# hyperplane-lab/ACL-GAN

Hardware: AMD Instinct MI355X
Metric: training images/sec at 256x256 (gen+dis step) (higher is better)
Workload: dtype fp32

## Files before the change

acl-gan_amd/csrc/conv_fast.hip:

```cpp
#include "conv_fast_common.h"
#include <cstring>

namespace aclgan {
namespace {


constexpr int BK = 16;
constexpr int WG_MAX_CHUNK = 1024 + 16;
constexpr int LDK = BK + 4;

template <int T, bool KC>
__device__ __forceinline__ void read_frags(const float* __restrict__ tile, int ld, int base, int lane, float (&f)[T][8]) {
    const int l31 = lane & 31, kh = lane >> 5;
    if (KC) {
#pragma unroll
        for (int t = 0; t < T; ++t) {
            const f32x4* p = reinterpret_cast<const f32x4*>(tile + (base + t * 32 + l31) * LDK + kh * 8);
            const f32x4 a = p[0], b = p[1];
            f[t][0] = a.x; f[t][1] = a.y; f[t][2] = a.z; f[t][3] = a.w;
            f[t][4] = b.x; f[t][5] = b.y; f[t][6] = b.z; f[t][7] = b.w;
        }
    } else {
#pragma unroll
        for (int ks = 0; ks < 8; ++ks)
#pragma unroll
            for (int t = 0; t < T; ++t) f[t][ks] = tile[(kh * 8 + ks) * ld + base + t * 32 + l31];
    }
}

template <int TM, int TN>
__device__ __forceinline__ void mfma_step(const float (&fa)[TM][8], const float (&fb)[TN][8], int ks, f32x16 (&acc)[TM][TN]) {
#pragma unroll
    for (int i = 0; i < TM; ++i)
#pragma unroll
        for (int j = 0; j < TN; ++j) acc[i][j] = __builtin_amdgcn_mfma_f32_32x32x2f32(fa[i][ks], fb[j][ks], acc[i][j], 0, 0, 0);
}

#define ACL_GEMM_MAINLOOP(TM_, TN_, AKC_, BKC_, KBEG_, NK_, AS_, BS_, ASTR_, BSTR_, LDA_, LDB_, AM_, BN_) \
    do {                                                                                                 \
        const int nk__ = (NK_), kb__ = (KBEG_);                                                          \
        fetch(kb__);                                                                                     \
        stage(0, true);                                                                                  \
        fetch(kb__ + min(1, nk__ - 1));                                                                  \
        __syncthreads();                                                                                 \
        for (int kt = 0; kt < nk__; ++kt) {                                                              \
            const int cur = kt & 1;                                                                      \
            float fa[TM_][8], fb[TN_][8];                                                                \
            read_frags<TM_, AKC_>((AS_) + cur * (ASTR_), (LDA_), (AM_), lane, fa);                       \
            read_frags<TN_, BKC_>((BS_) + cur * (BSTR_), (LDB_), (BN_), lane, fb);                       \
            if (!(AKC_) && !(BKC_)) __builtin_amdgcn_sched_barrier(0);    \
            mfma_step<TM_, TN_>(fa, fb, 0, acc);                                                         \
            stage(cur ^ 1, kt + 1 < nk__);                                                               \
            fetch(kb__ + min(kt + 2, nk__ - 1));                                                         \
            __builtin_amdgcn_sched_barrier(0x6);    \
            mfma_step<TM_, TN_>(fa, fb, 1, acc);                                                         \
            mfma_step<TM_, TN_>(fa, fb, 2, acc);                                                         \
            mfma_step<TM_, TN_>(fa, fb, 3, acc);                                                         \
            mfma_step<TM_, TN_>(fa, fb, 4, acc);                                                         \
            mfma_step<TM_, TN_>(fa, fb, 5, acc);                                                         \
            mfma_step<TM_, TN_>(fa, fb, 6, acc);                                                         \
            mfma_step<TM_, TN_>(fa, fb, 7, acc);                                                         \
            __syncthreads();                                                                             \
        }                                                                                                \
    } while (0)



template <int WM, int WN, int TM, int TN, int OCC = 1>
__global__ void __launch_bounds__(WM * WN * 64, OCC) conv_fwd_fast_kernel(FwdFP pk) {
    constexpr int BM = WM * TM * 32, BN = WN * TN * 32, NT = WM * WN * 64;
    constexpr int RP = NT / 4;
    FwdFP p = pk;
    if (pk.fsl) {
        const long long f = blockIdx.y;
        p.x += (pk.fsx_mod ? f % pk.fsx_mod : f) * pk.fs_x; p.w += f * pk.fs_w; p.y += f * pk.fs_y;
    }
    constexpr int A_IT = BM / RP, B_IT = (BN + RP - 1) / RP;
    __shared__ __attribute__((aligned(16))) float smem[2 * (BM + BN) * LDK];
    __shared__ int ro[BM];
    float* As = smem;
    float* Bs = smem + 2 * BM * LDK;

    const int tid = threadIdx.x, lane = tid & 63, wave = tid >> 6;
    const int wm = wave / WN, wn = wave % WN;
    const int tile = xcd_map(blockIdx.x, p.nwg);
    const int m0 = (tile / p.tiles_n) * BM, n0 = (tile % p.tiles_n) * BN;
    const int q = tid & 3, r0 = tid >> 2;
    const int phase = p.phases ? (int)blockIdx.z : 0;
    const float* wbase = p.w + (size_t)phase * p.Co * p.K;

    for (int r = tid; r < BM; r += NT) {
        int b, oy, ox, o = -1;
        if (fwd_row(p, m0 + r, b, oy, ox)) {
            if (p.phases) o = (b * p.Hf + 2 * (oy + 1) + (phase >> 1)) * p.Wf + 2 * (ox + 1) + (phase & 1);
            else o = (b * p.Ho + oy) * p.Wo + ox;
        }
        ro[r] = o;
    }
    int ay[A_IT], ax[A_IT], ab[A_IT];
#pragma unroll
    for (int i = 0; i < A_IT; ++i) {
        int b = 0, oy = 0, ox = 0;
        if (!fwd_row(p, m0 + r0 + i * RP, b, oy, ox)) { b = 0; oy = 0; ox = 0; }
        ay[i] = oy * p.s - p.p; ax[i] = ox * p.s - p.p; ab[i] = b * p.Hi * p.Wi;
    }
    int wo[B_IT];
#pragma unroll
    for (int i = 0; i < B_IT; ++i) wo[i] = min(n0 + r0 + i * RP, p.Co - 1) * p.K + q * 4;

    const int cpt = p.Ci >> 4;
    int aoff[A_IT];
    f32x4 ra[A_IT], rb[B_IT];
    int f_tap = -1;

    auto fetch = [&](int kt) __attribute__((always_inline)) {
        const int tap = kt / cpt, cc = kt - tap * cpt;
        if (tap != f_tap) {
            f_tap = tap;
            const int ky = tap / p.k, kx = tap - ky * p.k;
#pragma unroll
            for (int i = 0; i < A_IT; ++i) {
                const int iy = refl(ay[i] + ky, p.Hu) >> p.up;
                const int ix = refl(ax[i] + kx, p.Wu) >> p.up;
                aoff[i] = (ab[i] + iy * p.Wi + ix) * p.Ci + q * 4;
            }
        }
#pragma unroll
        for (int i = 0; i < A_IT; ++i) ra[i] = *reinterpret_cast<const f32x4*>(p.x + (size_t)aoff[i] + cc * 16);
#pragma unroll
        for (int i = 0; i < B_IT; ++i)
            if (BN % RP == 0 || r0 + i * RP < BN) rb[i] = *reinterpret_cast<const f32x4*>(wbase + (size_t)wo[i] + kt * 16);
    };
    auto stage = [&](int buf, bool real) __attribute__((always_inline)) {
        float* a = As + buf * BM * LDK;
        float* b = Bs + buf * BN * LDK;
#pragma unroll
        for (int i = 0; i < A_IT; ++i) *reinterpret_cast<f32x4*>(a + (r0 + i * RP) * LDK + q * 4) = ra[i];
#pragma unroll
        for (int i = 0; i < B_IT; ++i)
            if (BN % RP == 0 || r0 + i * RP < BN) *reinterpret_cast<f32x4*>(b + (r0 + i * RP) * LDK + q * 4) = rb[i];
    };

    f32x16 acc[TM][TN];
#pragma unroll
    for (int i = 0; i < TM; ++i)
#pragma unroll
        for (int j = 0; j < TN; ++j)
#pragma unroll
            for (int r = 0; r < 16; ++r) acc[i][j][r] = 0.f;

    const int nk_all = p.K / BK;
    const int kbeg = p.phases ? 0 : blockIdx.z * p.nkz, nk = p.phases ? nk_all : min(p.nkz, nk_all - kbeg);
    if (nk <= 0) return;
    const bool split = !p.phases && gridDim.z > 1;
    ACL_GEMM_MAINLOOP(TM, TN, true, true, kbeg, nk, As, Bs, BM * LDK, BN * LDK, LDK, LDK, wm * TM * 32, wn * TN * 32);

    const int l31 = lane & 31, lh = lane >> 5;
#pragma unroll
    for (int j = 0; j < TN; ++j) {
        const int n = n0 + wn * TN * 32 + j * 32 + l31;
        if (n >= p.Co) continue;
        const float bv = p.bias ? p.bias[n] : 0.f;
#pragma unroll
        for (int i = 0; i < TM; ++i) {
#pragma unroll
            for (int r = 0; r < 16; ++r) {
                const int rl = wm * TM * 32 + i * 32 + (r & 3) + 8 * (r >> 2) + 4 * lh;
                const int o = ro[rl];
                if (o >= 0) {
                    if (split && p.part) p.part[((size_t)blockIdx.z * p.rows + m0 + rl) * p.Co + n] = acc[i][j][r];
                    else if (split) atomicAdd(p.y + (size_t)o * p.Co + n, acc[i][j][r] + ((p.ring > 0 && blockIdx.z == 0) ? bv : 0.f));
                    else p.y[(size_t)o * p.Co + n] = act_apply(acc[i][j][r] + bv, p.act);
                }
            }
        }
    }
}


template <int WM, int WN, int TM, int TN>
int launch_fwd_fast(const ConvGeom& g, FwdFP p, hipStream_t st) {
    constexpr int BM = WM * TM * 32, BN = WN * TN * 32;
    p.tiles_n = cdiv(g.Co, BN);
    int rows = p.M;
    if (p.ring > 0) rows = p.B * (p.Ho * p.Wo - std::max(0, p.Ho - 2 * p.ring) * std::max(0, p.Wo - 2 * p.ring));
    p.nwg = cdiv(rows, BM) * p.tiles_n;
    if (p.phases) {
        hipLaunchKernelGGL((conv_fwd_fast_kernel<WM, WN, TM, TN>), dim3(p.nwg, 1, 4), dim3(WM * WN * 64), 0, st, p);
        ACL_CHECK_LAUNCH("conv_fwd_fast_kernel(phases)");
        return ACLGAN_OK;
    }
    int splits = 1;
    fwd_split_plan(rows, g.Co, g.K, BK, &splits, &p.nkz);
    p.rows = rows;
    if (splits > 1 && p.part != nullptr) {
        hipLaunchKernelGGL((conv_fwd_fast_kernel<WM, WN, TM, TN>), dim3(p.nwg, 1, splits), dim3(WM * WN * 64), 0, st, p);
        ACL_CHECK_LAUNCH("conv_fwd_fast_kernel(split)");
        hipLaunchKernelGGL(fwd_split_finish_kernel, dim3((int)std::min<int64_t>(cdiv64((int64_t)rows * std::max(1, g.Co / 4), 256), 4096)), dim3(256), 0, st, p, splits);
        ACL_CHECK_LAUNCH("fwd_split_finish_kernel");
        return ACLGAN_OK;
    }
    p.part = nullptr;
    const int nk = g.K / BK;
    if (p.ring > 0 && (p.act != ACLGAN_ACT_NONE || g.Co % 4 != 0)) splits = 1, p.nkz = nk;
    if (sw(SW_DETERMINISTIC)) splits = 1, p.nkz = nk;
    if (splits > 1 && p.ring > 0) {
        hipLaunchKernelGGL(ring_zero_kernel, dim3(cdiv(rows * (g.Co / 4), 256)), dim3(256), 0, st, p, rows);
        ACL_CHECK_LAUNCH("ring_zero_kernel");
    } else if (splits > 1) {
        hipError_t e = hipMemsetAsync(p.y, 0, (size_t)g.M * g.Co * sizeof(float), st);
        if (e != hipSuccess) return hip_fail(e, "memset y");
    }
    hipLaunchKernelGGL((conv_fwd_fast_kernel<WM, WN, TM, TN>), dim3(p.nwg, 1, splits), dim3(WM * WN * 64), 0, st, p);
    ACL_CHECK_LAUNCH("conv_fwd_fast_kernel");
    if (splits > 1 && p.ring == 0) {
        const int64_t n = (int64_t)g.M * g.Co;
        hipLaunchKernelGGL(bias_act_kernel, dim3((int)std::min<int64_t>(cdiv64(n, 256), 4096)), dim3(256), 0, st, p.y, p.bias, g.Co, p.act, n);
        ACL_CHECK_LAUNCH("bias_act_kernel");
    }
    return ACLGAN_OK;
}


template <int WM, int WN, int TM, int TN>
__global__ void __launch_bounds__(WM * WN * 64) conv_dgrad_fast_kernel(DgFP p) {
    constexpr int BM = WM * TM * 32, BN = WN * TN * 32, NT = WM * WN * 64;
    constexpr int RP = NT / 4;
    constexpr int A_IT = BM / RP;
    constexpr int LDB = BN + 4, NVB = BN / 4;
    constexpr int B_IT = (BK * NVB + NT - 1) / NT;
    __shared__ __attribute__((aligned(16))) float smem[2 * (BM * LDK + BK * LDB)];
    __shared__ int ri_o[BM];
    __shared__ unsigned long long tap_mask;
    __shared__ int tap_list[64];
    float* As = smem;
    float* Bs = smem + 2 * BM * LDK;

    const int tid = threadIdx.x, lane = tid & 63, wave = tid >> 6;
    const int wm = wave / WN, wn = wave % WN;
    const int tile = xcd_map(blockIdx.x, p.nwg);
    const int m0 = (tile / p.tiles_n) * BM;
    const int n0 = (tile % p.tiles_n) * BN;
    const int cls = blockIdx.z / p.ksplit, slice = blockIdx.z - cls * p.ksplit;
    const int cy = cls / p.s, cx = cls % p.s;
    const int Tx = (p.k - cx + p.s - 1) / p.s, Ty = (p.k - cy + p.s - 1) / p.s;
    const int q = tid & 3, r0 = tid >> 2;

    int ylo, yhi, xlo, xhi;
    dg_box(p, cy, cx, ylo, yhi, xlo, xhi);
    const bool compact = p.mode == 2 && Ty * Tx <= 64;
    if (tid == 0) tap_mask = 0ull;
    __syncthreads();
    for (int r = tid; r < BM; r += NT) {
        int oo = -1, b, y2, x2;
        if (dg_row(p, m0 + r, ylo, yhi, xlo, xhi, b, y2, x2)) {
            const int py = y2 * p.s + cy, px = x2 * p.s + cx;
            if (compact && py < p.Hp && px < p.Wp) {
                unsigned long long mk = 0ull;
                for (int t = 0; t < Ty * Tx; ++t) {
                    const int ty = t / Tx, tx = t - ty * Tx;
                    const int oy = y2 - ty, ox = x2 - tx;
                    bool ok = (unsigned)oy < (unsigned)p.Ho && (unsigned)ox < (unsigned)p.Wo;
                    if (p.band > 0) ok = ok && (oy < 2 || oy >= p.Ho - 2 || ox < 2 || ox >= p.Wo - 2);
                    if (ok) mk |= 1ull << t;
                }
                if (mk) atomicOr(&tap_mask, mk);
            }
            if (py < p.Hp && px < p.Wp) {
                if (p.mode == 0 || p.ringpad) oo = (b * p.Hp + py) * p.Wp + px;
                else oo = (b * p.Hd + (refl(py - p.pad, p.Hi) >> p.upshift)) * p.Wd + (refl(px - p.pad, p.Wi) >> p.upshift);
            }
        }
        ri_o[r] = oo;
    }
    int ntap = Ty * Tx;
    if (compact) {
        __syncthreads();
        if (tid == 0) {
            int n = 0;
            for (int t = 0; t < Ty * Tx; ++t)
                if ((tap_mask >> t) & 1ull) tap_list[n++] = t;
            tap_list[63] = n;
        }
        __syncthreads();
        ntap = tap_list[63];
        if (ntap == 0) return;
    }
    int ay[A_IT], ax[A_IT], ab[A_IT];
#pragma unroll
    for (int i = 0; i < A_IT; ++i) {
        int b = 0, y2 = 0, x2 = 0;
        if (!dg_row(p, m0 + r0 + i * RP, ylo, yhi, xlo, xhi, b, y2, x2)) { b = 0; y2 = 0; x2 = 0; }
        ay[i] = y2; ax[i] = x2; ab[i] = b;
    }
    int bo[B_IT];
#pragma unroll
    for (int i = 0; i < B_IT; ++i) {
        const int idx = tid + i * NT;
        const int krow = idx / NVB, nc = idx - krow * NVB;
        const int n = n0 + nc * 4;
        bo[i] = krow * p.k * p.k * p.Ci + (n < p.Ci ? n : 0);
    }
    const int cpt = p.Co >> 4;
    int aoff[A_IT];
    f32x4 ra[A_IT], rb[B_IT];
    float za[A_IT];
    int f_tap = -1, tapoff = 0;

    auto fetch = [&](int kt) __attribute__((always_inline)) {
        const int tq = kt / cpt, cc = kt - tq * cpt;
        if (tq != f_tap) {
            f_tap = tq;
            const int t = compact ? tap_list[tq] : tq;
            const int ty = t / Tx, tx = t - ty * Tx;
            tapoff = ((cy + p.s * ty) * p.k + (cx + p.s * tx)) * p.Ci;
#pragma unroll
            for (int i = 0; i < A_IT; ++i) {
                const int oy = ay[i] - ty, ox = ax[i] - tx;
                const bool ok = (unsigned)oy < (unsigned)p.Ho && (unsigned)ox < (unsigned)p.Wo;
                bool okk = ok;
                if (p.band > 0) okk = ok && (oy < 2 || oy >= p.Ho - 2 || ox < 2 || ox >= p.Wo - 2);
                const int dpix = p.dyv ? (ab[i] * p.Hf + 2 * (oy + 1) + p.py) * p.Wf + 2 * (ox + 1) + p.px
                                       : (ab[i] * p.Ho + oy) * p.Wo + ox;
                aoff[i] = okk ? dpix * p.Co + q * 4 : -1;
            }
        }
#pragma unroll
        for (int i = 0; i < A_IT; ++i) {
            ra[i] = *reinterpret_cast<const f32x4*>(p.dy + (size_t)(aoff[i] < 0 ? 0 : aoff[i]) + cc * 16);
            za[i] = aoff[i] < 0 ? 0.f : 1.f;
        }
#pragma unroll
        for (int i = 0; i < B_IT; ++i)
            if ((BK * NVB) % NT == 0 || tid + i * NT < BK * NVB)
                rb[i] = *reinterpret_cast<const f32x4*>(p.w + (size_t)bo[i] + tapoff + (size_t)cc * 16 * p.k * p.k * p.Ci);
    };
    auto stage = [&](int buf, bool real) __attribute__((always_inline)) {
        float* a = As + buf * BM * LDK;
        float* b = Bs + buf * BK * LDB;
#pragma unroll
        for (int i = 0; i < A_IT; ++i) *reinterpret_cast<f32x4*>(a + (r0 + i * RP) * LDK + q * 4) = ra[i] * za[i];
#pragma unroll
        for (int i = 0; i < B_IT; ++i) {
            const int idx = tid + i * NT;
            if ((BK * NVB) % NT == 0 || idx < BK * NVB) {
                const int krow = idx / NVB, nc = idx - krow * NVB;
                *reinterpret_cast<f32x4*>(b + krow * LDB + nc * 4) = rb[i];
            }
        }
    };

    f32x16 acc[TM][TN];
#pragma unroll
    for (int i = 0; i < TM; ++i)
#pragma unroll
        for (int j = 0; j < TN; ++j)
#pragma unroll
            for (int r = 0; r < 16; ++r) acc[i][j][r] = 0.f;

    const int nk_all = ntap * cpt;
    const int nkz = (nk_all + p.ksplit - 1) / p.ksplit;
    const int kbeg = slice * nkz, nk = min(nkz, nk_all - kbeg);
    if (nk <= 0) return;
    ACL_GEMM_MAINLOOP(TM, TN, true, false, kbeg, nk, As, Bs, BM * LDK, BK * LDB, LDK, LDB, wm * TM * 32, wn * TN * 32);

    const int l31 = lane & 31, lh = lane >> 5;
#pragma unroll
    for (int j = 0; j < TN; ++j) {
        const int n = n0 + wn * TN * 32 + j * 32 + l31;
        if (n >= p.Ci) continue;
#pragma unroll
        for (int i = 0; i < TM; ++i) {
#pragma unroll
            for (int r = 0; r < 16; ++r) {
                const int of = ri_o[wm * TM * 32 + i * 32 + (r & 3) + 8 * (r >> 2) + 4 * lh];
                if (of >= 0) {
                    float* o = p.dxp + (size_t)of * p.Ci + n;
                    if (p.ksplit > 1 || (p.mode == 2 && !p.ringpad)) atomicAdd(o, acc[i][j][r]);
                    else if (p.accumulate) *o += acc[i][j][r];
                    else *o = acc[i][j][r];
                }
            }
        }
    }
}

template <int WM, int WN, int TM, int TN>
int launch_dgrad_fast(const ConvGeom& g, DgFP p, hipStream_t st) {
    constexpr int BM = WM * TM * 32, BN = WN * TN * 32;
    int mmax = 0;
    for (int cy = 0; cy < g.s; ++cy)
        for (int cx = 0; cx < g.s; ++cx) {
            const int ylo = g.p > cy ? (g.p - cy + g.s - 1) / g.s : 0, xlo = g.p > cx ? (g.p - cx + g.s - 1) / g.s : 0;
            const int yhi = std::min(p.Hc - 1, (g.p + g.Hi - 1 - cy) / g.s), xhi = std::min(p.Wc - 1, (g.p + g.Wi - 1 - cx) / g.s);
            int inner = (yhi - ylo + 1) * (xhi - xlo + 1);
            if (p.band > 0) inner = std::max(0, p.Hc - 2 * p.band) * std::max(0, p.Wc - 2 * p.band);
            const int rows = p.mode == 0 ? p.Hc * p.Wc : (p.mode == 1 ? inner : p.Hc * p.Wc - inner);
            mmax = std::max(mmax, g.B * rows);
        }
    if (mmax <= 0) return ACLGAN_OK;
    p.Mc = mmax;
    p.tiles_n = cdiv(g.Ci, BN);
    p.nwg = cdiv(p.Mc, BM) * p.tiles_n;
    const int nk_min = ((g.k + g.s - 1) / g.s) * ((g.k + g.s - 1) / g.s) * (g.Co / 16);
    const int nblk = p.nwg * g.s * g.s;
    p.ksplit = 1;
    const int nk_plan = (p.mode == 2 && p.band == 0) ? std::max(g.Co / 16, nk_min / ((g.k + g.s - 1) / g.s)) : nk_min;
    if (nblk < 128 && nk_plan >= 32 && !sw(SW_DETERMINISTIC) && !p.ringpad)
        p.ksplit = max(1, min(nk_plan / 8, 512 / nblk));
    if (p.ksplit > 1 && p.mode == 0) {
        hipError_t e = hipMemsetAsync(p.dxp, 0, conv_dgrad_scratch_bytes(g), st);
        if (e != hipSuccess) return hip_fail(e, "memset dxp");
    }
    if (p.ksplit > 1 && p.mode == 1 && !p.accumulate) {
        hipError_t e = hipMemsetAsync(p.dxp, 0, (size_t)g.B * g.Hi * g.Wi * g.Ci * sizeof(float), st);
        if (e != hipSuccess) return hip_fail(e, "memset dx");
    }
    hipLaunchKernelGGL((conv_dgrad_fast_kernel<WM, WN, TM, TN>), dim3(p.nwg, 1, g.s * g.s * p.ksplit), dim3(WM * WN * 64), 0, st, p);
    ACL_CHECK_LAUNCH("conv_dgrad_fast_kernel");
    return ACLGAN_OK;
}

template <int WM, int WN, int TM, int TN>
int launch_dgrad_halo(const ConvGeom& g, DgFP p, hipStream_t st) {
    if (p.band == 0 && !p.ringpad && g.k == 3 && g.s == 1 && g.Ci % 128 == 0 && WM == 2 && WN == 2 && TM == 2 && TN == 2)
        return launch_dgrad_fast<2, 2, 1, 2>(g, p, st);
    return launch_dgrad_fast<WM, WN, TM, TN>(g, p, st);
}

template <int WM, int WN, int TM, int TN>
int dgrad_fast_all(const ConvGeom& g, DgFP p, float* dxp, float* dx, int accumulate, bool* direct, hipStream_t st) {
    if (g.up == 0 && dx != nullptr && (!sw(SW_DETERMINISTIC) || g.p == 0 || (dxp && conv_wino_ok(g)))) {
        *direct = true;
        p.dxp = dx; p.accumulate = accumulate;
        p.mode = 1;
        int rc = (dxp && conv_wino_ok(g)) ? conv_dgrad_wino_interior(g, p.dy, p.w, dx, accumulate, dxp, st)
             : (dxp && conv_s2k4_wino_ok(g, 1)) ? conv_dgrad_s2k4_wino_interior(g, p.dy, p.w, dx, accumulate, dxp, st)
                                      : launch_dgrad_fast<WM, WN, TM, TN>(g, p, st);
        if (rc) return rc;
        if (g.p > 0 && sw(SW_DETERMINISTIC)) {
            hipError_t e = hipMemsetAsync(dxp, 0, (size_t)g.B * g.Hp * g.Wp * g.Ci * sizeof(float), st);
            if (e != hipSuccess) return hip_fail(e, "memset padded grid");
            p.mode = 2; p.ringpad = 1; p.dxp = dxp; p.accumulate = 0;
            rc = launch_dgrad_fast<WM, WN, TM, TN>(g, p, st);
            if (rc) return rc;
            return conv_fold(g, dxp, dx, 1, st);
        }
        if (g.p > 0) { p.mode = 2; rc = launch_dgrad_halo<WM, WN, TM, TN>(g, p, st); }
        return rc;
    }
    *direct = false;
    p.dxp = dxp; p.mode = 0; p.accumulate = 0;
    return launch_dgrad_fast<WM, WN, TM, TN>(g, p, st);
}


template <int WM, int WN, int TM, int TN, bool ST>
__global__ void __launch_bounds__(WM * WN * 64) conv_wgrad_fast_kernel(WgFP p) {
    constexpr int BM = WM * TM * 32, BN = WN * TN * 32, NT = WM * WN * 64;
    constexpr int LDA = BM + 4, LDB = BN + 4, MVA = BM / 4, NVB = BN / 4;
    constexpr int A_IT = (BK * MVA + NT - 1) / NT, B_IT = (BK * NVB + NT - 1) / NT;
    __shared__ __attribute__((aligned(16))) float smem[2 * BK * (LDA + LDB)];
    float* As = smem;
    float* Bs = smem + 2 * BK * LDA;

    const int tid = threadIdx.x, lane = tid & 63, wave = tid >> 6;
    const int wm = wave / WN, wn = wave % WN;
    const int tile = xcd_map(blockIdx.x, p.nwg);
    const int m0 = (tile / p.tiles_n) * BM, n0 = (tile % p.tiles_n) * BN;
    const int pbeg = blockIdx.z * p.chunk;
    const int pend = min(p.P, pbeg + p.chunk);
    if (pbeg >= pend) return;
    const int phase = p.phases ? (int)blockIdx.y : 0;
    float* dwbase = p.dw + (size_t)phase * p.Co * p.Kn + (size_t)blockIdx.z * p.dw_zs;
    const int py = phase >> 1, px = phase & 1;

    __shared__ int4 pinfo[WG_MAX_CHUNK];
    const int st_tap = n0 / p.Ci, st_ky = st_tap / p.k, st_kx = st_tap - st_ky * p.k;
    for (int i = tid; i < pend - pbeg + BK; i += NT) {
        int b, oy, ox;
        wg_coord(p, min(pbeg + i, pend - 1), b, oy, ox);
        const int dyp = p.phases ? (b * p.Hf + 2 * (oy + 1) + py) * p.Wf + 2 * (ox + 1) + px : (b * p.Ho + oy) * p.Wo + ox;
        if (ST) {
            const int iy = refl(oy * p.s - p.p + st_ky, p.Hu) >> p.up, ix = refl(ox * p.s - p.p + st_kx, p.Wu) >> p.up;
            pinfo[i] = make_int4(b * p.Hi * p.Wi + iy * p.Wi + ix, 0, 0, dyp);
        } else {
            pinfo[i] = make_int4(oy * p.s - p.p, ox * p.s - p.p, b * p.Hi * p.Wi, dyp);
        }
    }
    __syncthreads();

    int a_m[A_IT], a_kr[A_IT];
#pragma unroll
    for (int i = 0; i < A_IT; ++i) {
        const int idx = tid + i * NT;
        a_kr[i] = idx / MVA;
        const int m = m0 + (idx - a_kr[i] * MVA) * 4;
        a_m[i] = m < p.Co ? m : 0;
    }
    int b_kr[B_IT], b_ci[B_IT], b_ky[B_IT], b_kx[B_IT];
#pragma unroll
    for (int i = 0; i < B_IT; ++i) {
        const int idx = tid + i * NT;
        b_kr[i] = idx / NVB;
        int n = n0 + (idx - b_kr[i] * NVB) * 4;
        if (n >= p.Kn) n = 0;
        const int tap = n / p.Ci;
        b_ci[i] = n - tap * p.Ci; b_ky[i] = tap / p.k; b_kx[i] = tap - b_ky[i] * p.k;
    }
    f32x4 ra[A_IT], rb[B_IT];
    float za[A_IT];
    const bool do_bias = p.db != nullptr && (tile % p.tiles_n) == 0;
    f32x4 bsum[A_IT];
#pragma unroll
    for (int i = 0; i < A_IT; ++i) bsum[i] = (f32x4){0.f, 0.f, 0.f, 0.f};

    auto fetch = [&](int kt) __attribute__((always_inline)) {
        const int pb = kt * BK;
#pragma unroll
        for (int i = 0; i < A_IT; ++i) {
            if ((BK * MVA) % NT != 0 && tid + i * NT >= BK * MVA) continue;
            const int pi = pb + a_kr[i];
            ra[i] = *reinterpret_cast<const f32x4*>(p.dy + (size_t)pinfo[pi].w * p.Co + a_m[i]);
            za[i] = pbeg + pi < pend ? 1.f : 0.f;
        }
#pragma unroll
        for (int i = 0; i < B_IT; ++i) {
            if ((BK * NVB) % NT != 0 && tid + i * NT >= BK * NVB) continue;
            if (ST) {
                rb[i] = *reinterpret_cast<const f32x4*>(p.x + (size_t)pinfo[pb + b_kr[i]].x * p.Ci + b_ci[i]);
            } else {
                const int4 pi = pinfo[pb + b_kr[i]];
                const int iy = refl(pi.x + b_ky[i], p.Hu) >> p.up;
                const int ix = refl(pi.y + b_kx[i], p.Wu) >> p.up;
                rb[i] = *reinterpret_cast<const f32x4*>(p.x + (size_t)(pi.z + iy * p.Wi + ix) * p.Ci + b_ci[i]);
            }
        }
    };
    auto stage = [&](int buf, bool real) __attribute__((always_inline)) {
        float* a = As + buf * BK * LDA;
        float* b = Bs + buf * BK * LDB;
#pragma unroll
        for (int i = 0; i < A_IT; ++i) {
            const int idx = tid + i * NT;
            if ((BK * MVA) % NT == 0 || idx < BK * MVA) {
                const f32x4 v = ra[i] * za[i];
                *reinterpret_cast<f32x4*>(a + a_kr[i] * LDA + (idx - a_kr[i] * MVA) * 4) = v;
                bsum[i] += v * (real ? 1.f : 0.f);
            }
        }
#pragma unroll
        for (int i = 0; i < B_IT; ++i) {
            const int idx = tid + i * NT;
            if ((BK * NVB) % NT == 0 || idx < BK * NVB) *reinterpret_cast<f32x4*>(b + b_kr[i] * LDB + (idx - b_kr[i] * NVB) * 4) = rb[i];
        }
    };

    f32x16 acc[TM][TN];
#pragma unroll
    for (int i = 0; i < TM; ++i)
#pragma unroll
        for (int j = 0; j < TN; ++j)
#pragma unroll
            for (int r = 0; r < 16; ++r) acc[i][j][r] = 0.f;

    ACL_GEMM_MAINLOOP(TM, TN, false, false, 0, (pend - pbeg + BK - 1) / BK, As, Bs, BK * LDA, BK * LDB, LDA, LDB, wm * TM * 32, wn * TN * 32);

    if (do_bias) {
        float* red = smem;
#pragma unroll
        for (int i = 0; i < A_IT; ++i) {
            const int idx = tid + i * NT;
            if ((BK * MVA) % NT == 0 || idx < BK * MVA) *reinterpret_cast<f32x4*>(red + a_kr[i] * BM + (idx - a_kr[i] * MVA) * 4) = bsum[i];
        }
        __syncthreads();
        if (tid < BM && m0 + tid < p.Co) {
            float t = 0.f;
#pragma unroll
            for (int r = 0; r < BK; ++r) t += red[r * BM + tid];
            atomicAdd(p.db + (size_t)blockIdx.z * p.db_zs + m0 + tid, t);
        }
    }
    const int l31 = lane & 31, lh = lane >> 5;
#pragma unroll
    for (int j = 0; j < TN; ++j) {
        const int n = n0 + wn * TN * 32 + j * 32 + l31;
        if (n >= p.Kn) continue;
#pragma unroll
        for (int i = 0; i < TM; ++i) {
#pragma unroll
            for (int r = 0; r < 16; ++r) {
                const int m = m0 + wm * TM * 32 + i * 32 + (r & 3) + 8 * (r >> 2) + 4 * lh;
                if (m < p.Co) {
                    atomicAdd(dwbase + (size_t)m * p.Kn + n, acc[i][j][r]);
                }
            }
        }
    }
}

constexpr int WGKC_TARGET = 768;

template <int WM, int WN, int TM, int TN>
__global__ void __launch_bounds__(WM * WN * 64) conv_wgrad_kc_kernel(WgFP pk, WgPartX xp) {
    constexpr int BM = WM * TM * 32, BN = WN * TN * 32, NT = WM * WN * 64;
    WgFP p = pk;
    if (pk.fsl) {
        const long long f = blockIdx.y;
        p.x += (pk.fsx_mod ? f % pk.fsx_mod : f) * pk.fs_x; p.dy += f * pk.fs_dy;
    }
    static_assert(BM % 64 == 0 && BN % 64 == 0 && BM + BN <= NT, "one staging unit (4 channels x 4 pixels) per thread, wave-uniform roles");
    constexpr int CH = 1024;
    __shared__ __attribute__((aligned(16))) float smem[2 * (BM + BN) * LDK];
    __shared__ int2 pinfo[CH + BK];
    float* As = smem;
    float* Bs = smem + 2 * BM * LDK;

    const int tid = threadIdx.x, lane = tid & 63, wave = tid >> 6;
    const int wm = wave / WN, wn = wave % WN;
    const int tile = xcd_map(blockIdx.x, p.nwg);
    const int m0 = (tile / p.tiles_n) * BM, n0 = (tile % p.tiles_n) * BN;
    const int pbeg = blockIdx.z * p.chunk;
    const int pend = min(p.P, pbeg + p.chunk);
    const int phase = (p.phases || p.fsl) ? (int)blockIdx.y : 0;
    float* dwbase = p.dw + (size_t)phase * p.Co * p.Kn;
    const int py = phase >> 1, px = phase & 1;
    const int st_tap = n0 / p.Ci, st_ky = st_tap / p.k, st_kx = st_tap - st_ky * p.k;

    const bool isA = tid < BM, isB = !isA && tid < BM + BN;
    const int u = isA ? tid : tid - BM;
    const int ncg = (isA ? BM : BN) >> 2;
    const int cg = u % ncg, pg = u / ncg;
    const float* src = isA ? p.dy : p.x;
    const int cstride = isA ? p.Co : p.Ci;
    const int chan = isA ? m0 + 4 * cg : (n0 - st_tap * p.Ci) + 4 * cg;
    float* mytile = isA ? As : Bs;
    const int tstride = (isA ? BM : BN) * LDK;
    f32x4 rr[4];
    float zm[4];
    const bool do_bias = p.db != nullptr && (tile % p.tiles_n) == 0;
    f32x4 bsum = {0.f, 0.f, 0.f, 0.f};

    f32x16 acc[TM][TN];
#pragma unroll
    for (int i = 0; i < TM; ++i)
#pragma unroll
        for (int j = 0; j < TN; ++j)
#pragma unroll
            for (int r = 0; r < 16; ++r) acc[i][j][r] = 0.f;

    for (int cb = pbeg; cb < pend; cb += CH) {
        const int ce = min(pend, cb + CH);
        for (int i = tid; i < ce - cb + BK; i += NT) {
            int b, oy, ox;
            wg_coord(p, min(cb + i, ce - 1), b, oy, ox);
            const int dyp = p.phases ? (b * p.Hf + 2 * (oy + 1) + py) * p.Wf + 2 * (ox + 1) + px : (b * p.Ho + oy) * p.Wo + ox;
            const int iy = refl(oy * p.s - p.p + st_ky, p.Hu) >> p.up, ix = refl(ox * p.s - p.p + st_kx, p.Wu) >> p.up;
            pinfo[i] = make_int2(b * p.Hi * p.Wi + iy * p.Wi + ix, dyp);
        }
        __syncthreads();

        auto fetch = [&](int kt) __attribute__((always_inline)) {
            const int pb = kt * BK + 4 * pg;
            if (isA || isB) {
#pragma unroll
                for (int j = 0; j < 4; ++j) {
                    const int2 pi = pinfo[pb + j];
                    rr[j] = *reinterpret_cast<const f32x4*>(src + (size_t)(isA ? pi.y : pi.x) * cstride + chan);
                    zm[j] = cb + pb + j < ce ? 1.f : 0.f;
                }
            }
        };
        auto stage = [&](int buf, bool real) __attribute__((always_inline)) {
            if (isA || isB) {
                float* t = mytile + buf * tstride;
                f32x4 v[4];
#pragma unroll
                for (int j = 0; j < 4; ++j) v[j] = rr[j] * zm[j];
                if (isA) {
                    const float on = real ? 1.f : 0.f;
#pragma unroll
                    for (int j = 0; j < 4; ++j) bsum += v[j] * on;
                }
#pragma unroll
                for (int c = 0; c < 4; ++c) {
                    const f32x4 k4 = {v[0][c], v[1][c], v[2][c], v[3][c]};
                    *reinterpret_cast<f32x4*>(t + (c * ncg + cg) * LDK + 4 * pg) = k4;
                }
            }
        };
        ACL_GEMM_MAINLOOP(TM, TN, true, true, 0, (ce - cb + BK - 1) / BK, As, Bs, BM * LDK, BN * LDK, LDK, LDK, wm * TM * 32, wn * TN * 32);
    }

    const bool partial = xp.part != nullptr;
    if (do_bias) {
        float* red = smem;
        if (isA) *reinterpret_cast<f32x4*>(red + pg * BM + 4 * cg) = bsum;
        __syncthreads();
        if (tid < BM) {
            const float t = red[tid] + red[BM + tid] + red[2 * BM + tid] + red[3 * BM + tid];
            if (partial) xp.part_b[((size_t)blockIdx.z * xp.ny + phase) * p.Co + m0 + tid] = t;
            else p.db[m0 + tid] += t;
        }
    }
    const int l31 = lane & 31, lh = lane >> 5;
    constexpr int MQ = BM / 4, NQ = BN / 4;
    if (partial) {
        float* pt = xp.part + (((size_t)blockIdx.z * xp.ny + phase) * p.nwg + tile) * (BM * BN);
#pragma unroll
        for (int j = 0; j < TN; ++j)
#pragma unroll
            for (int i = 0; i < TM; ++i)
#pragma unroll
                for (int r = 0; r < 16; ++r) {
                    const int rw = wm * TM * 32 + i * 32 + (r & 3) + 8 * (r >> 2) + 4 * lh;
                    pt[rw * BN + wn * TN * 32 + j * 32 + l31] = acc[i][j][r];
                }
        return;
    }
#pragma unroll
    for (int j = 0; j < TN; ++j) {
        const int cr = wn * TN * 32 + j * 32 + l31;
        const int n = n0 + 4 * (cr % NQ) + cr / NQ;
#pragma unroll
        for (int i = 0; i < TM; ++i) {
#pragma unroll
            for (int r = 0; r < 16; ++r) {
                const int rw = wm * TM * 32 + i * 32 + (r & 3) + 8 * (r >> 2) + 4 * lh;
                const int m = m0 + 4 * (rw % MQ) + rw / MQ;
                dwbase[(size_t)m * p.Kn + n] += acc[i][j][r];
            }
        }
    }
}

bool wgrad_kc_ok(const ConvGeom& g) {
    return !sw(SW_NOWGKC) && g.Co % 64 == 0 && g.Ci % 64 == 0;
}

template <int WM, int WN, int TM, int TN>
int launch_wgrad_kc(const ConvGeom& g, WgFP p, void* part, hipStream_t st) {
    constexpr int BM = WM * TM * 32, BN = WN * TN * 32;
    const int ny = p.fsl ? p.fsl : (p.phases ? 4 : 1);
    const WgPlan q = wgrad_plan(g.Co, p.Ci, p.Kn, p.P, ny, BK, WGKC_TARGET);
// ... 364 lines not shown
```

acl-gan_amd/csrc/switches.h:

```cpp
#pragma once
#include <atomic>

namespace aclgan {

enum SwitchId {
    SW_LANES, SW_U_BATCH, SW_NORM_MASK, SW_MLP_FUSED, SW_FAULT_AT, SW_ENC_REUSE,
    SW_GLDS_TILE, SW_WINO_X3, SW_WINO_FUSED, SW_WINO_WGRAD_FUSED, SW_WINO_S2K4, SW_DGRAD16S_DIRECT, SW_FWD16_PATCH,
    SW_DETERMINISTIC,
    SW_NOFAST, SW_NOUP5, SW_SPLIT_NWG,
    SW_NOWGKC, SW_NOUP5DGRAD,
    SW_NOSTATFUSE, SW_NOKEEPV, SW_NODIRECT,
    SW_NOWGRAD16S, SW_WGRAD16S_MINPIX, SW_NOGLDS16,
    SW_NOSMALL, SW_NOTHIN,
    SW_NOWINO, SW_NOWINOUP5, SW_WINO_VEC, SW_WINO_VEC3,
    SW_ROCTX, SW_NOUCACHE, SW_ACT16, SW_CO16, SW_SIDE_STREAM, SW_KEEPV_BUDGET_GB,
    SW_COUNT
};

const long long SW_BIAS = 1ll << 32;
extern std::atomic<long long> g_switches[SW_COUNT];
int sw_latch(SwitchId id);
inline int sw(SwitchId id) {
    const long long e = g_switches[id].load(std::memory_order_relaxed);
    return e ? (int)(e - SW_BIAS) : sw_latch(id);
}
double sw_real(SwitchId id);
int sw_set(SwitchId id, int v);

long long tuning_epoch();

}
```

acl-gan_amd/csrc/switches.hip:

```cpp
#include <string.h>
#include "common.h"

#include <climits>
#include <cmath>
#include <cstdlib>

namespace aclgan {

namespace {

enum Rule {
    R_INT,
    R_BOOL,
    R_NOT,
    R_CLAMP,
    R_RANGE,
    R_LOW4,
    R_ONEOF,
};
enum { SETTABLE = 1,
       EMPTY_UNSET = 2 };

struct Switch {
    const char* key;
    const char* env;
    int dflt;
    Rule rule;
    int lo, hi;
    int flags;
    double (*parse)(const char*);
};

double parse_real(const char* s) { return atof(s); }
const int VEC_124 = (1 << 1) | (1 << 2) | (1 << 4);

const Switch kSwitches[SW_COUNT] = {
    {"lanes",             "ACLGAN_LANES",             3,  R_CLAMP, 1, 3,       SETTABLE | EMPTY_UNSET, nullptr},
    {"u_batch",           "ACLGAN_U_BATCH",           1,  R_BOOL,  0, 0,       SETTABLE | EMPTY_UNSET, nullptr},
    {"norm_mask",         "ACLGAN_NORM_MASK",         1,  R_BOOL,  0, 0,       SETTABLE | EMPTY_UNSET, nullptr},
    {"mlp_fused",         "ACLGAN_MLP_FUSED",         1,  R_BOOL,  0, 0,       SETTABLE | EMPTY_UNSET, nullptr},
    {"fault_at",          nullptr,                    -1, R_INT,   0, 0,       SETTABLE, nullptr},
    {"enc_reuse",         nullptr,                    1,  R_BOOL,  0, 0,       SETTABLE, nullptr},
    {"glds_tile",         "ACLGAN_GLDS_TILE",         0,  R_CLAMP, 0, INT_MAX, SETTABLE, nullptr},
    {"wino_x3",           "ACLGAN_WINO_X3",           0,  R_BOOL,  0, 0,       SETTABLE, nullptr},
    {"wino_fused",        "ACLGAN_WINO_FUSED",        1,  R_LOW4,  0, 2,       SETTABLE, nullptr},
    {"wino_wgrad_fused",  "ACLGAN_WINO_WGRAD_FUSED",  1,  R_RANGE, 0, 2,       SETTABLE, nullptr},
    {"wino_s2k4",         "ACLGAN_NOWINOS2",          1,  R_NOT,   0, 0,       SETTABLE, nullptr},
    {"dgrad16s_direct",   "ACLGAN_DGRAD16S_DIRECT",   0,  R_BOOL,  0, 0,       SETTABLE, nullptr},
    {"fwd16_patch",       "ACLGAN_FWD16_PATCH",       1,  R_LOW4,  0, 2,       SETTABLE, nullptr},
    {"deterministic",     "ACLGAN_DETERMINISTIC",     0,  R_BOOL,  0, 0,       0, nullptr},
    {"nofast",            "ACLGAN_NOFAST",            0,  R_BOOL,  0, 0,       0, nullptr},
    {"noup5",             "ACLGAN_NOUP5",             0,  R_BOOL,  0, 0,       0, nullptr},
    {"split_nwg",         "ACLGAN_SPLIT_NWG",         256, R_INT,  0, 0,       0, nullptr},
    {"nowgkc",            "ACLGAN_NOWGKC",            0,  R_BOOL,  0, 0,       0, nullptr},
    {"noup5dgrad",        "ACLGAN_NOUP5DGRAD",        0,  R_BOOL,  0, 0,       0, nullptr},
    {"nostatfuse",        "ACLGAN_NOSTATFUSE",        0,  R_BOOL,  0, 0,       0, nullptr},
    {"nokeepv",           "ACLGAN_NOKEEPV",           0,  R_BOOL,  0, 0,       0, nullptr},
    {"nodirect",          "ACLGAN_NODIRECT",          0,  R_BOOL,  0, 0,       0, nullptr},
    {"nowgrad16s",        "ACLGAN_NOWGRAD16S",        0,  R_BOOL,  0, 0,       0, nullptr},
    {"wgrad16s_minpix",   "ACLGAN_WGRAD16S_MINPIX",   64, R_INT,   0, 0,       0, nullptr},
    {"noglds16",          "ACLGAN_NOGLDS16",          0,  R_BOOL,  0, 0,       0, nullptr},
    {"nosmall",           "ACLGAN_NOSMALL",           0,  R_BOOL,  0, 0,       0, nullptr},
    {"nothin",            "ACLGAN_NOTHIN",            0,  R_BOOL,  0, 0,       0, nullptr},
    {"nowino",            "ACLGAN_NOWINO",            0,  R_BOOL,  0, 0,       0, nullptr},
    {"nowinoup5",         "ACLGAN_NOWINOUP5",         0,  R_BOOL,  0, 0,       0, nullptr},
    {"wino_vec",          "ACLGAN_WINO_VEC",          2,  R_ONEOF, VEC_124, 0, 0, nullptr},
    {"wino_vec3",         "ACLGAN_WINO_VEC3",         2,  R_ONEOF, VEC_124, 0, 0, nullptr},
    {"roctx",             "ACLGAN_ROCTX",             0,  R_BOOL,  0, 0,       0, nullptr},
    {"noucache",          "ACLGAN_NOUCACHE",          0,  R_BOOL,  0, 0,       0, nullptr},
    {"act16",             "ACLGAN_ACT16",             1,  R_BOOL,  0, 0,       0, nullptr},
    {"co16",              "ACLGAN_CO16",              1,  R_BOOL,  0, 0,       0, nullptr},
    {"side_stream",       "ACLGAN_SIDE_STREAM",       1,  R_BOOL,  0, 0,       0, nullptr},
    {"keepv_budget_gb",   "ACLGAN_KEEPV_BUDGET_GB",   64, R_INT,   0, 0,       0, parse_real},
};

int normalise(const Switch& s, int v, bool from_env) {
    switch (s.rule) {
    case R_INT: return v;
    case R_BOOL: return v ? 1 : 0;
    case R_NOT: return (v ? 1 : 0) ^ (from_env ? 1 : 0);
    case R_CLAMP: return v < s.lo ? s.lo : v > s.hi ? s.hi : v;
    case R_RANGE: return (v < s.lo || v > s.hi) ? s.dflt : v;
    case R_LOW4: return (v < 0 || (v & 15) < s.lo || (v & 15) > s.hi) ? s.dflt : v;
    case R_ONEOF: return (v >= 0 && v < 31 && ((s.lo >> v) & 1)) ? v : s.dflt;
    }
    return v;
}

std::atomic<double> g_real[SW_COUNT];
std::atomic<long long> g_tuning_epoch{0};

int find(const char* key) {
    for (int i = 0; i < SW_COUNT; ++i)
        if (!strcmp(key, kSwitches[i].key)) return i;
    return -1;
}

}

std::atomic<long long> g_switches[SW_COUNT];

int sw_latch(SwitchId id) {
// ... 64 lines not shown
```

Baseline: 103.8.

## Add deeper register prefetch for fwd/dgrad conv GEMM on small grids

Makes the shared GEMM main loop templated on a prefetch depth. The fwd and dgrad conv kernels can now keep several k-tiles of global loads in flight in register sets while still using a double-buffered LDS. Depth 2 is chosen by default when the grid is at most the CU count, or when split-K grids are small, so latency is hidden better where occupancy is low. The cost is extra VGPRs per thread, which could lower occupancy or cause spills, plus more template instantiations. Ablation macros and a settable switch are added for sweeping.

```diff
diff --git a/acl-gan_amd/csrc/conv_fast.hip b/acl-gan_amd/csrc/conv_fast.hip
--- a/acl-gan_amd/csrc/conv_fast.hip
+++ b/acl-gan_amd/csrc/conv_fast.hip
@@ -28,45 +28,65 @@
     }
 }
 
+#ifndef ACLGAN_LOOP_ABLATION
+#define ACLGAN_LOOP_ABLATION 0
+#endif
+
 template <int TM, int TN>
 __device__ __forceinline__ void mfma_step(const float (&fa)[TM][8], const float (&fb)[TN][8], int ks, f32x16 (&acc)[TM][TN]) {
 #pragma unroll
     for (int i = 0; i < TM; ++i)
 #pragma unroll
-        for (int j = 0; j < TN; ++j) acc[i][j] = __builtin_amdgcn_mfma_f32_32x32x2f32(fa[i][ks], fb[j][ks], acc[i][j], 0, 0, 0);
-}
-
-#define ACL_GEMM_MAINLOOP(TM_, TN_, AKC_, BKC_, KBEG_, NK_, AS_, BS_, ASTR_, BSTR_, LDA_, LDB_, AM_, BN_) \
+        for (int j = 0; j < TN; ++j) {
+            if (ACLGAN_LOOP_ABLATION & 1) asm volatile("" :: "v"(fa[i][ks]), "v"(fb[j][ks]));
+            else acc[i][j] = __builtin_amdgcn_mfma_f32_32x32x2f32(fa[i][ks], fb[j][ks], acc[i][j], 0, 0, 0);
+        }
+}
+
+#define ACL_GEMM_KTILE(J_, D_, TM_, TN_, AKC_, BKC_, AS_, BS_, ASTR_, BSTR_, LDA_, LDB_, AM_, BN_)       \
+    if ((J_) < (D_)) {                                                                                   \
+        const int kt = kt0__ + (J_);                                                                     \
+        if ((J_) > 0 && kt >= nk__) break;                                                               \
+        const int cur = kt & 1;                                                                          \
+        float fa[TM_][8], fb[TN_][8];                                                                    \
+        read_frags<TM_, AKC_>((AS_) + cur * (ASTR_), (LDA_), (AM_), lane, fa);                           \
+        read_frags<TN_, BKC_>((BS_) + cur * (BSTR_), (LDB_), (BN_), lane, fb);                           \
+        if (!(AKC_) && !(BKC_)) __builtin_amdgcn_sched_barrier(0);    \
+        mfma_step<TM_, TN_>(fa, fb, 0, acc);                                                             \
+        if (!(ACLGAN_LOOP_ABLATION & 4)) stage(cur ^ 1, kt + 1 < nk__, ((J_) + 1) % (D_));               \
+        if (!(ACLGAN_LOOP_ABLATION & 2)) fetch(kb__ + min(kt + (1 + (D_)), nk__ - 1), ((J_) + 1) % (D_)); \
+        __builtin_amdgcn_sched_barrier(0x6);    \
+        mfma_step<TM_, TN_>(fa, fb, 1, acc);                                                             \
+        mfma_step<TM_, TN_>(fa, fb, 2, acc);                                                             \
+        mfma_step<TM_, TN_>(fa, fb, 3, acc);                                                             \
+        mfma_step<TM_, TN_>(fa, fb, 4, acc);                                                             \
+        mfma_step<TM_, TN_>(fa, fb, 5, acc);                                                             \
+        mfma_step<TM_, TN_>(fa, fb, 6, acc);                                                             \
+        mfma_step<TM_, TN_>(fa, fb, 7, acc);                                                             \
+        if (!(ACLGAN_LOOP_ABLATION & 4)) __syncthreads();                                                \
+    }
+#define ACL_GEMM_MAINLOOP(D_, TM_, TN_, AKC_, BKC_, KBEG_, NK_, AS_, BS_, ASTR_, BSTR_, LDA_, LDB_, AM_, BN_) \
     do {                                                                                                 \
+        static_assert((D_) >= 1 && (D_) <= 4, "prefetch depth 1 .. 4");                                  \
         const int nk__ = (NK_), kb__ = (KBEG_);                                                          \
-        fetch(kb__);                                                                                     \
-        stage(0, true);                                                                                  \
-        fetch(kb__ + min(1, nk__ - 1));                                                                  \
+        fetch(kb__, 0);                                                                                  \
+        if ((D_) > 1) fetch(kb__ + min(1, nk__ - 1), 1 % (D_));                                          \
+        if ((D_) > 2) fetch(kb__ + min(2, nk__ - 1), 2 % (D_));                                          \
+        if ((D_) > 3) fetch(kb__ + min(3, nk__ - 1), 3 % (D_));                                          \
+        stage(0, true, 0);                                                                               \
+        fetch(kb__ + min((D_), nk__ - 1), 0);                                                            \
         __syncthreads();                                                                                 \
-        for (int kt = 0; kt < nk__; ++kt) {                                                              \
-            const int cur = kt & 1;                                                                      \
-            float fa[TM_][8], fb[TN_][8];                                                                \
-            read_frags<TM_, AKC_>((AS_) + cur * (ASTR_), (LDA_), (AM_), lane, fa);                       \
-            read_frags<TN_, BKC_>((BS_) + cur * (BSTR_), (LDB_), (BN_), lane, fb);                       \
-            if (!(AKC_) && !(BKC_)) __builtin_amdgcn_sched_barrier(0);    \
-            mfma_step<TM_, TN_>(fa, fb, 0, acc);                                                         \
-            stage(cur ^ 1, kt + 1 < nk__);                                                               \
-            fetch(kb__ + min(kt + 2, nk__ - 1));                                                         \
-            __builtin_amdgcn_sched_barrier(0x6);    \
-            mfma_step<TM_, TN_>(fa, fb, 1, acc);                                                         \
-            mfma_step<TM_, TN_>(fa, fb, 2, acc);                                                         \
-            mfma_step<TM_, TN_>(fa, fb, 3, acc);                                                         \
-            mfma_step<TM_, TN_>(fa, fb, 4, acc);                                                         \
-            mfma_step<TM_, TN_>(fa, fb, 5, acc);                                                         \
-            mfma_step<TM_, TN_>(fa, fb, 6, acc);                                                         \
-            mfma_step<TM_, TN_>(fa, fb, 7, acc);                                                         \
-            __syncthreads();                                                                             \
+        for (int kt0__ = 0; kt0__ < nk__; kt0__ += (D_)) {                                               \
+            ACL_GEMM_KTILE(0, D_, TM_, TN_, AKC_, BKC_, AS_, BS_, ASTR_, BSTR_, LDA_, LDB_, AM_, BN_)    \
+            ACL_GEMM_KTILE(1, D_, TM_, TN_, AKC_, BKC_, AS_, BS_, ASTR_, BSTR_, LDA_, LDB_, AM_, BN_)    \
+            ACL_GEMM_KTILE(2, D_, TM_, TN_, AKC_, BKC_, AS_, BS_, ASTR_, BSTR_, LDA_, LDB_, AM_, BN_)    \
+            ACL_GEMM_KTILE(3, D_, TM_, TN_, AKC_, BKC_, AS_, BS_, ASTR_, BSTR_, LDA_, LDB_, AM_, BN_)    \
         }                                                                                                \
     } while (0)
 
 
 
-template <int WM, int WN, int TM, int TN, int OCC = 1>
+template <int WM, int WN, int TM, int TN, int OCC = 1, int PD = 1>
 __global__ void __launch_bounds__(WM * WN * 64, OCC) conv_fwd_fast_kernel(FwdFP pk) {
     constexpr int BM = WM * TM * 32, BN = WN * TN * 32, NT = WM * WN * 64;
     constexpr int RP = NT / 4;
@@ -110,10 +130,10 @@
 
     const int cpt = p.Ci >> 4;
     int aoff[A_IT];
-    f32x4 ra[A_IT], rb[B_IT];
+    f32x4 ra[PD][A_IT], rb[PD][B_IT];
     int f_tap = -1;
 
-    auto fetch = [&](int kt) __attribute__((always_inline)) {
+    auto fetch = [&](int kt, int set) __attribute__((always_inline)) {
         const int tap = kt / cpt, cc = kt - tap * cpt;
         if (tap != f_tap) {
             f_tap = tap;
@@ -126,19 +146,19 @@
             }
         }
 #pragma unroll
-        for (int i = 0; i < A_IT; ++i) ra[i] = *reinterpret_cast<const f32x4*>(p.x + (size_t)aoff[i] + cc * 16);
+        for (int i = 0; i < A_IT; ++i) ra[set][i] = *reinterpret_cast<const f32x4*>(p.x + (size_t)aoff[i] + cc * 16);
 #pragma unroll
         for (int i = 0; i < B_IT; ++i)
-            if (BN % RP == 0 || r0 + i * RP < BN) rb[i] = *reinterpret_cast<const f32x4*>(wbase + (size_t)wo[i] + kt * 16);
+            if (BN % RP == 0 || r0 + i * RP < BN) rb[set][i] = *reinterpret_cast<const f32x4*>(wbase + (size_t)wo[i] + kt * 16);
     };
-    auto stage = [&](int buf, bool real) __attribute__((always_inline)) {
+    auto stage = [&](int buf, bool real, int set) __attribute__((always_inline)) {
         float* a = As + buf * BM * LDK;
         float* b = Bs + buf * BN * LDK;
 #pragma unroll
-        for (int i = 0; i < A_IT; ++i) *reinterpret_cast<f32x4*>(a + (r0 + i * RP) * LDK + q * 4) = ra[i];
+        for (int i = 0; i < A_IT; ++i) *reinterpret_cast<f32x4*>(a + (r0 + i * RP) * LDK + q * 4) = ra[set][i];
 #pragma unroll
         for (int i = 0; i < B_IT; ++i)
-            if (BN % RP == 0 || r0 + i * RP < BN) *reinterpret_cast<f32x4*>(b + (r0 + i * RP) * LDK + q * 4) = rb[i];
+            if (BN % RP == 0 || r0 + i * RP < BN) *reinterpret_cast<f32x4*>(b + (r0 + i * RP) * LDK + q * 4) = rb[set][i];
     };
 
     f32x16 acc[TM][TN];
@@ -153,7 +173,7 @@
     const int kbeg = p.phases ? 0 : blockIdx.z * p.nkz, nk = p.phases ? nk_all : min(p.nkz, nk_all - kbeg);
     if (nk <= 0) return;
     const bool split = !p.phases && gridDim.z > 1;
-    ACL_GEMM_MAINLOOP(TM, TN, true, true, kbeg, nk, As, Bs, BM * LDK, BN * LDK, LDK, LDK, wm * TM * 32, wn * TN * 32);
+    ACL_GEMM_MAINLOOP(PD, TM, TN, true, true, kbeg, nk, As, Bs, BM * LDK, BN * LDK, LDK, LDK, wm * TM * 32, wn * TN * 32);
 
     const int l31 = lane & 31, lh = lane >> 5;
 #pragma unroll
@@ -177,6 +197,31 @@
     }
 }
 
+
+#ifdef ACLGAN_PREFETCH_SWEEP
+constexpr int PD_MAX = 4;
+#else
+constexpr int PD_MAX = 2;
+#endif
+constexpr int PD_SMALL_GRID = 2;
+constexpr int NUM_CU = 256;
+int prefetch_depth(int nblk, int slices) {
+    const int v = sw(SW_PREFETCH);
+    if (v >= 1) return std::min(v, PD_MAX);
+    return (nblk <= NUM_CU || (slices > 1 && nblk <= 2 * NUM_CU)) ? PD_SMALL_GRID : 1;
+}
+
+template <int WM, int WN, int TM, int TN>
+void fwd_fast_go(int depth, dim3 grid, const FwdFP& p, hipStream_t st) {
+    switch (depth) {
+    case 2: hipLaunchKernelGGL((conv_fwd_fast_kernel<WM, WN, TM, TN, 1, 2>), grid, dim3(WM * WN * 64), 0, st, p); break;
+#ifdef ACLGAN_PREFETCH_SWEEP
+    case 3: hipLaunchKernelGGL((conv_fwd_fast_kernel<WM, WN, TM, TN, 1, 3>), grid, dim3(WM * WN * 64), 0, st, p); break;
+    case 4: hipLaunchKernelGGL((conv_fwd_fast_kernel<WM, WN, TM, TN, 1, 4>), grid, dim3(WM * WN * 64), 0, st, p); break;
+#endif
+    default: hipLaunchKernelGGL((conv_fwd_fast_kernel<WM, WN, TM, TN>), grid, dim3(WM * WN * 64), 0, st, p);
+    }
+}
 
 template <int WM, int WN, int TM, int TN>
 int launch_fwd_fast(const ConvGeom& g, FwdFP p, hipStream_t st) {
@@ -194,7 +239,7 @@
     fwd_split_plan(rows, g.Co, g.K, BK, &splits, &p.nkz);
     p.rows = rows;
     if (splits > 1 && p.part != nullptr) {
-        hipLaunchKernelGGL((conv_fwd_fast_kernel<WM, WN, TM, TN>), dim3(p.nwg, 1, splits), dim3(WM * WN * 64), 0, st, p);
+        fwd_fast_go<WM, WN, TM, TN>(prefetch_depth(p.nwg * splits, splits), dim3(p.nwg, 1, splits), p, st);
         ACL_CHECK_LAUNCH("conv_fwd_fast_kernel(split)");
         hipLaunchKernelGGL(fwd_split_finish_kernel, dim3((int)std::min<int64_t>(cdiv64((int64_t)rows * std::max(1, g.Co / 4), 256), 4096)), dim3(256), 0, st, p, splits);
         ACL_CHECK_LAUNCH("fwd_split_finish_kernel");
@@ -211,7 +256,7 @@
         hipError_t e = hipMemsetAsync(p.y, 0, (size_t)g.M * g.Co * sizeof(float), st);
         if (e != hipSuccess) return hip_fail(e, "memset y");
     }
-    hipLaunchKernelGGL((conv_fwd_fast_kernel<WM, WN, TM, TN>), dim3(p.nwg, 1, splits), dim3(WM * WN * 64), 0, st, p);
+    fwd_fast_go<WM, WN, TM, TN>(prefetch_depth(p.nwg * splits, splits), dim3(p.nwg, 1, splits), p, st);
     ACL_CHECK_LAUNCH("conv_fwd_fast_kernel");
     if (splits > 1 && p.ring == 0) {
         const int64_t n = (int64_t)g.M * g.Co;
@@ -222,7 +267,7 @@
 }
 
 
-template <int WM, int WN, int TM, int TN>
+template <int WM, int WN, int TM, int TN, int PD = 1>
 __global__ void __launch_bounds__(WM * WN * 64) conv_dgrad_fast_kernel(DgFP p) {
     constexpr int BM = WM * TM * 32, BN = WN * TN * 32, NT = WM * WN * 64;
     constexpr int RP = NT / 4;
@@ -303,11 +348,11 @@
     }
     const int cpt = p.Co >> 4;
     int aoff[A_IT];
-    f32x4 ra[A_IT], rb[B_IT];
-    float za[A_IT];
+    f32x4 ra[PD][A_IT], rb[PD][B_IT];
+    float za[PD * A_IT];
     int f_tap = -1, tapoff = 0;
 
-    auto fetch = [&](int kt) __attribute__((always_inline)) {
+    auto fetch = [&](int kt, int set) __attribute__((always_inline)) {
         const int tq = kt / cpt, cc = kt - tq * cpt;
         if (tq != f_tap) {
             f_tap = tq;
@@ -327,25 +372,25 @@
         }
 #pragma unroll
         for (int i = 0; i < A_IT; ++i) {
-            ra[i] = *reinterpret_cast<const f32x4*>(p.dy + (size_t)(aoff[i] < 0 ? 0 : aoff[i]) + cc * 16);
-            za[i] = aoff[i] < 0 ? 0.f : 1.f;
+            ra[set][i] = *reinterpret_cast<const f32x4*>(p.dy + (size_t)(aoff[i] < 0 ? 0 : aoff[i]) + cc * 16);
+            za[set * A_IT + i] = aoff[i] < 0 ? 0.f : 1.f;
         }
 #pragma unroll
         for (int i = 0; i < B_IT; ++i)
             if ((BK * NVB) % NT == 0 || tid + i * NT < BK * NVB)
-                rb[i] = *reinterpret_cast<const f32x4*>(p.w + (size_t)bo[i] + tapoff + (size_t)cc * 16 * p.k * p.k * p.Ci);
+                rb[set][i] = *reinterpret_cast<const f32x4*>(p.w + (size_t)bo[i] + tapoff + (size_t)cc * 16 * p.k * p.k * p.Ci);
     };
-    auto stage = [&](int buf, bool real) __attribute__((always_inline)) {
+    auto stage = [&](int buf, bool real, int set) __attribute__((always_inline)) {
         float* a = As + buf * BM * LDK;
         float* b = Bs + buf * BK * LDB;
 #pragma unroll
-        for (int i = 0; i < A_IT; ++i) *reinterpret_cast<f32x4*>(a + (r0 + i * RP) * LDK + q * 4) = ra[i] * za[i];
+        for (int i = 0; i < A_IT; ++i) *reinterpret_cast<f32x4*>(a + (r0 + i * RP) * LDK + q * 4) = ra[set][i] * za[set * A_IT + i];
 #pragma unroll
         for (int i = 0; i < B_IT; ++i) {
             const int idx = tid + i * NT;
             if ((BK * NVB) % NT == 0 || idx < BK * NVB) {
                 const int krow = idx / NVB, nc = idx - krow * NVB;
-                *reinterpret_cast<f32x4*>(b + krow * LDB + nc * 4) = rb[i];
+                *reinterpret_cast<f32x4*>(b + krow * LDB + nc * 4) = rb[set][i];
             }
         }
     };
@@ -362,7 +407,7 @@
     const int nkz = (nk_all + p.ksplit - 1) / p.ksplit;
     const int kbeg = slice * nkz, nk = min(nkz, nk_all - kbeg);
     if (nk <= 0) return;
-    ACL_GEMM_MAINLOOP(TM, TN, true, false, kbeg, nk, As, Bs, BM * LDK, BK * LDB, LDK, LDB, wm * TM * 32, wn * TN * 32);
+    ACL_GEMM_MAINLOOP(PD, TM, TN, true, false, kbeg, nk, As, Bs, BM * LDK, BK * LDB, LDK, LDB, wm * TM * 32, wn * TN * 32);
 
     const int l31 = lane & 31, lh = lane >> 5;
 #pragma unroll
@@ -416,7 +461,15 @@
         hipError_t e = hipMemsetAsync(p.dxp, 0, (size_t)g.B * g.Hi * g.Wi * g.Ci * sizeof(float), st);
         if (e != hipSuccess) return hip_fail(e, "memset dx");
     }
-    hipLaunchKernelGGL((conv_dgrad_fast_kernel<WM, WN, TM, TN>), dim3(p.nwg, 1, g.s * g.s * p.ksplit), dim3(WM * WN * 64), 0, st, p);
+    const dim3 grid(p.nwg, 1, g.s * g.s * p.ksplit);
+    switch (prefetch_depth(nblk * p.ksplit, p.ksplit)) {
+    case 2: hipLaunchKernelGGL((conv_dgrad_fast_kernel<WM, WN, TM, TN, 2>), grid, dim3(WM * WN * 64), 0, st, p); break;
+#ifdef ACLGAN_PREFETCH_SWEEP
+    case 3: hipLaunchKernelGGL((conv_dgrad_fast_kernel<WM, WN, TM, TN, 3>), grid, dim3(WM * WN * 64), 0, st, p); break;
+    case 4: hipLaunchKernelGGL((conv_dgrad_fast_kernel<WM, WN, TM, TN, 4>), grid, dim3(WM * WN * 64), 0, st, p); break;
+#endif
+    default: hipLaunchKernelGGL((conv_dgrad_fast_kernel<WM, WN, TM, TN>), grid, dim3(WM * WN * 64), 0, st, p);
+    }
     ACL_CHECK_LAUNCH("conv_dgrad_fast_kernel");
     return ACLGAN_OK;
 }
@@ -515,7 +568,7 @@
 #pragma unroll
     for (int i = 0; i < A_IT; ++i) bsum[i] = (f32x4){0.f, 0.f, 0.f, 0.f};
 
-    auto fetch = [&](int kt) __attribute__((always_inline)) {
+    auto fetch = [&](int kt, int) __attribute__((always_inline)) {
         const int pb = kt * BK;
 #pragma unroll
         for (int i = 0; i < A_IT; ++i) {
@@ -537,7 +590,7 @@
             }
         }
     };
-    auto stage = [&](int buf, bool real) __attribute__((always_inline)) {
+    auto stage = [&](int buf, bool real, int) __attribute__((always_inline)) {
         float* a = As + buf * BK * LDA;
         float* b = Bs + buf * BK * LDB;
 #pragma unroll
@@ -564,7 +617,7 @@
 #pragma unroll
             for (int r = 0; r < 16; ++r) acc[i][j][r] = 0.f;
 
-    ACL_GEMM_MAINLOOP(TM, TN, false, false, 0, (pend - pbeg + BK - 1) / BK, As, Bs, BK * LDA, BK * LDB, LDA, LDB, wm * TM * 32, wn * TN * 32);
+    ACL_GEMM_MAINLOOP(1, TM, TN, false, false, 0, (pend - pbeg + BK - 1) / BK, As, Bs, BK * LDA, BK * LDB, LDA, LDB, wm * TM * 32, wn * TN * 32);
 
     if (do_bias) {
         float* red = smem;
@@ -660,7 +713,7 @@
         }
         __syncthreads();
 
-        auto fetch = [&](int kt) __attribute__((always_inline)) {
+        auto fetch = [&](int kt, int) __attribute__((always_inline)) {
             const int pb = kt * BK + 4 * pg;
             if (isA || isB) {
 #pragma unroll
@@ -671,7 +724,7 @@
                 }
             }
         };
-        auto stage = [&](int buf, bool real) __attribute__((always_inline)) {
+        auto stage = [&](int buf, bool real, int) __attribute__((always_inline)) {
             if (isA || isB) {
                 float* t = mytile + buf * tstride;
                 f32x4 v[4];
@@ -689,7 +742,7 @@
                 }
             }
         };
-        ACL_GEMM_MAINLOOP(TM, TN, true, true, 0, (ce - cb + BK - 1) / BK, As, Bs, BM * LDK, BN * LDK, LDK, LDK, wm * TM * 32, wn * TN * 32);
+        ACL_GEMM_MAINLOOP(1, TM, TN, true, true, 0, (ce - cb + BK - 1) / BK, As, Bs, BM * LDK, BN * LDK, LDK, LDK, wm * TM * 32, wn * TN * 32);
     }
 
     const bool partial = xp.part != nullptr;
diff --git a/acl-gan_amd/csrc/switches.h b/acl-gan_amd/csrc/switches.h
--- a/acl-gan_amd/csrc/switches.h
+++ b/acl-gan_amd/csrc/switches.h
@@ -5,7 +5,7 @@
 
 enum SwitchId {
     SW_LANES, SW_U_BATCH, SW_NORM_MASK, SW_MLP_FUSED, SW_FAULT_AT, SW_ENC_REUSE,
-    SW_GLDS_TILE, SW_WINO_X3, SW_WINO_FUSED, SW_WINO_WGRAD_FUSED, SW_WINO_S2K4, SW_DGRAD16S_DIRECT, SW_FWD16_PATCH,
+    SW_GLDS_TILE, SW_WINO_X3, SW_WINO_FUSED, SW_WINO_WGRAD_FUSED, SW_WINO_S2K4, SW_DGRAD16S_DIRECT, SW_FWD16_PATCH, SW_PREFETCH,
     SW_DETERMINISTIC,
     SW_NOFAST, SW_NOUP5, SW_SPLIT_NWG,
     SW_NOWGKC, SW_NOUP5DGRAD,
diff --git a/acl-gan_amd/csrc/switches.hip b/acl-gan_amd/csrc/switches.hip
--- a/acl-gan_amd/csrc/switches.hip
+++ b/acl-gan_amd/csrc/switches.hip
@@ -48,6 +48,7 @@
     {"wino_s2k4",         "ACLGAN_NOWINOS2",          1,  R_NOT,   0, 0,       SETTABLE, nullptr},
     {"dgrad16s_direct",   "ACLGAN_DGRAD16S_DIRECT",   0,  R_BOOL,  0, 0,       SETTABLE, nullptr},
     {"fwd16_patch",       "ACLGAN_FWD16_PATCH",       1,  R_LOW4,  0, 2,       SETTABLE, nullptr},
+    {"prefetch",          nullptr,                    0,  R_RANGE, 0, 4,       SETTABLE, nullptr},
     {"deterministic",     "ACLGAN_DETERMINISTIC",     0,  R_BOOL,  0, 0,       0, nullptr},
     {"nofast",            "ACLGAN_NOFAST",            0,  R_BOOL,  0, 0,       0, nullptr},
     {"noup5",             "ACLGAN_NOUP5",             0,  R_BOOL,  0, 0,       0, nullptr},
```

New measurement: 103.8 (median of 4 runs). Within noise of the previous version (+0.0%).
